# nnnagle/vq-vae

Measured on AMD Instinct MI355X. Metric: tiles/sec, higher is better.
Workload: dtype bf16

## Files before the change

### include/frl_hip.h

```cpp
#ifndef FRL_HIP_H
#define FRL_HIP_H

#include <stddef.h>
#include <stdint.h>

#ifdef __cplusplus
extern "C" {
#endif

typedef void* frl_stream_t;

enum { FRL_F32 = 0, FRL_BF16 = 1, FRL_F16 = 2  };
enum { FRL_ACT_NONE = 0, FRL_ACT_RELU = 1, FRL_ACT_SIGMOID = 2 };

int frl_version(void);
const char* frl_last_error(void);
int frl_device_arch(char* buf, int n);
int frl_kernel_timing_enable(int on);
int frl_kernel_timing_report(char* buf, int n);

size_t frl_pack_cache_table_bytes(void);
int frl_pack_cache_create(void* arena, size_t bytes);
int frl_pack_cache_destroy(int handle);
int frl_pack_cache_activate(int handle);
int frl_pack_cache_images(int handle);
int frl_pack_cache_refresh(int handle, frl_stream_t stream);

size_t frl_conv_workspace_bytes(int Cin, int Cout, int taps);
int frl_conv1x1_fwd(const void* x, const float* w, const float* bias, void* y, int64_t P, int Cin, int Cout, int act,
                    int dtype, void* ws, size_t ws_bytes, frl_stream_t stream);
int frl_conv1x1_bwd_data(const void* dy, const void* y, int act, const float* w, void* dx, int64_t P, int Cin, int Cout,
                         int dtype, void* ws, size_t ws_bytes, frl_stream_t stream);
int frl_conv1x1_bwd_data_add(const void* dy, const void* y, int act, const float* w, void* dx, const void* add, int64_t P,
                             int Cin, int Cout, int dtype, void* ws, size_t ws_bytes, frl_stream_t stream);
int frl_wgrad_set_max_workgroups(int n);
size_t frl_conv1x1_bwd_weight_workspace_bytes(int64_t P, int Cin, int Cout);
int frl_conv1x1_bwd_weight(const void* dy, const void* y, int act, const void* x, float* dw, float* dbias, int64_t P,
                           int Cin, int Cout, int dtype, void* ws, size_t ws_bytes, frl_stream_t stream);
int frl_conv_tap_bwd_weight(const void* dy, const void* y, int act, const void* x, float* dw, int64_t dso, int64_t dsi,
                            float* dbias, int64_t P, int Cin, int Cout, int HW, int T, int toff, int dtype, void* ws,
                            size_t ws_bytes, int flags, frl_stream_t stream);

int frl_conv3x3_fwd(const void* x, const float* w, const float* bias, void* y, int B, int H, int W, int Cin, int Cout,
                    int act, int dtype, void* ws, size_t ws_bytes, frl_stream_t stream);
int frl_conv3x3_fwd_gate_blend(const void* x, const float* w, const float* bias, const void* smoothed, const void* residual, void* gate,
                               void* out, int B, int H, int W, int Cin, int Cout, int dtype, void* ws, size_t ws_bytes,
                               frl_stream_t stream);
int frl_conv3x3_bwd_data(const void* dy, const void* y, int act, const float* w, void* dx, int B, int H, int W, int Cin,
                         int Cout, int dtype, void* ws, size_t ws_bytes, frl_stream_t stream);
int frl_conv3x3_bwd_data_fused(const void* dy, const void* y, int act, const float* w, void* dx, const void* add,
                               const void* sub_from, void* out2, int B, int H, int W, int Cin, int Cout, int dtype, void* ws,
                               size_t ws_bytes, frl_stream_t stream);
int frl_conv3x3_bwd_data_outmask(const void* dy, const void* y, int act, const float* w, void* dx, const void* out_y, int out_act, int B,
                                 int H, int W, int Cin, int Cout, int dtype, void* ws, size_t ws_bytes, frl_stream_t stream);
size_t frl_conv3x3_bwd_weight_workspace_bytes(int B, int H, int W, int Cin, int Cout);
int frl_conv3x3_bwd_weight(const void* dy, const void* y, int act, const void* x, float* dw, float* dbias, int B, int H,
                           int W, int Cin, int Cout, int dtype, void* ws, size_t ws_bytes, int flags, frl_stream_t stream);
int frl_conv3x3_wgrad_force_generic(int on);
int frl_conv3x3_tile32(int on);

int frl_groupnorm_fwd(const void* x, const float* gamma, const float* beta, void* y, float* mean, float* rstd, int B,
                      int HW, int C, int G, float eps, int relu, int dtype, frl_stream_t stream);
size_t frl_groupnorm_bwd_workspace_bytes(int B, int C, int G);
int frl_groupnorm_bwd(const void* dy, const void* x, const float* gamma, const float* beta, const float* mean,
                      const float* rstd, void* dx, float* dgamma, float* dbeta, int B, int HW, int C, int G, int relu,
                      int dtype, void* ws, size_t ws_bytes, frl_stream_t stream);

int frl_scalar_combine(const float* const* terms_host, const float* coef_host, int n, float* out, float* ok_out, frl_stream_t stream);
int frl_scalar_fanout(const float* g, const float* coef_host, int n, float* out, frl_stream_t stream);
int frl_scalar_combine_dev(const float* const* terms_host, const float* coef_host, const float* const* mult_host, int n, float* out,
                           float* ok_out, frl_stream_t stream);
int frl_scalar_combine_aux(const float* const* terms_host, const float* coef_host, const float* const* mult_host, const float* aux_coef_host,
                           int n, float* out, float* ok_out, float* aux_out, frl_stream_t stream);
int frl_scalar_fanout_dev(const float* g, const float* coef_host, const float* const* mult_host, int n, float* out, frl_stream_t stream);
int frl_scalar_fanout_guard(const float* g, const float* coef_host, const float* const* mult_host, const float* const* promise_host, int n,
                            float* out, int* flag, frl_stream_t stream);

int frl_encoder2_supported(int C0, int C1, int C2, int G1, int G2, int HW, int dtype);
size_t frl_encoder2_workspace_bytes(int B);
int frl_encoder2_fwd(const void* x, const float* w1, const float* g1, const float* b1, const float* w2, const float* g2, const float* b2,
                     void* z, float* stats, int B, int HW, float eps, void* ws, size_t ws_bytes, frl_stream_t stream);
int frl_encoder2_bwd(const void* x, const void* dz, const float* w1, const float* g1, const float* b1, const float* w2, const float* g2,
                     const float* b2, const float* stats, float* dw1, float* dg1, float* db1, float* dw2, float* dg2, float* db2,
                     int B, int HW, void* ws, size_t ws_bytes, frl_stream_t stream);

int frl_sobel_fwd(const void* x, void* g, int B, int H, int W, int C, int dtype, frl_stream_t stream);
int frl_sobel_bwd(const void* dg, void* dx, int B, int H, int W, int C, int dtype, frl_stream_t stream);
int frl_sobel_bwd_add(const void* dg, void* dx, const void* dx_add, int B, int H, int W, int C, int dtype, frl_stream_t stream);
int frl_edge_smooth_stencil_fwd(const void* x, const void* a_logit, const void* b_logit, void* smoothed, void* residual,
                                void* a_soft, void* b_soft, int B, int H, int W, int C, int R, int coarse_dilation,
                                int dtype, frl_stream_t stream);
int frl_edge_smooth_stencil_bwd(const void* d_smoothed, const void* x, const void* a_soft, const void* b_soft, void* dx,
                                void* da_logit, void* db_logit, const void* dx_add , int B, int H,
                                int W, int C, int R, int coarse_dilation, int dtype, frl_stream_t stream);
int frl_smooth_heads_supported(int C, int hidden, int rank, int dtype);
size_t frl_smooth_heads_workspace_bytes(int64_t npix);
int frl_smooth_heads_fwd(const void* x, const void* feat, const float* wa, const float* ba, const float* wb, const float* bb,
                         void* smoothed, void* residual, int B, int H, int W, int coarse_dilation, void* ws, size_t ws_bytes,
                         frl_stream_t stream);
size_t frl_smooth_heads_bwd_scratch_bytes(int64_t npix);
int frl_smooth_heads_force_gather(int on);
int frl_smooth_heads_bwd(const void* d_smoothed, const void* x, const void* feat, const float* wa, const float* ba, const float* wb,
                         const float* bb, const void* dx_add, void* dx, void* dfeat, float* dwa, float* dba, float* dwb, float* dbb,
                         void* scratch, size_t scratch_bytes, int B, int H, int W, int coarse_dilation, void* ws, size_t ws_bytes,
                         frl_stream_t stream);
int frl_smooth_heads_bwd_masked(const void* d_smoothed, const void* x, const void* feat, const float* wa, const float* ba, const float* wb,
                                const float* bb, const void* dx_add, void* dx, void* dfeat, float* dwa, float* dba, float* dwb, float* dbb,
                                void* scratch, size_t scratch_bytes, int B, int H, int W, int dil, int dfeat_relu, void* ws,
                                size_t ws_bytes, frl_stream_t stream);
int frl_film_fused_supported(int cond_dim, int hidden, int target_dim, int dtype);
size_t frl_film_fused_workspace_bytes(void);
int frl_film_fused_fwd(const void* z_type, const void* h, const float* w1g, const float* b1g, const float* w2g, const float* b2g,
                       const float* w1b, const float* b1b, const float* w2b, const float* b2b, void* z, void* gamma, void* beta, int B,
                       int T, int HW, void* ws, size_t ws_bytes, frl_stream_t stream);
int frl_film_fused_bwd(const void* z_type, const void* h, const void* dz, const float* w1g, const float* b1g, const float* w2g,
                       const float* b2g, const float* w1b, const float* b1b, const float* w2b, const float* b2b, void* dh, float* dw1g,
                       float* db1g, float* dw2g, float* db2g, float* dw1b, float* db1b, float* dw2b, float* db2b, int B, int T, int HW,
                       void* ws, size_t ws_bytes, frl_stream_t stream);
int frl_gate_blend_fwd(const void* smoothed, const void* residual, const void* gate_raw, float min_gate, void* out,
                       void* gate_out, int64_t n, int dtype, frl_stream_t stream);
int frl_gate_blend_bwd(const void* dout, const void* dgate_ext, const void* residual, const void* gate_raw, float min_gate,
                       void* d_residual, void* d_gate_raw, int64_t n, int dtype, frl_stream_t stream);
int frl_gate_blend_bwd_masked(const void* dout, const void* dgate_ext, const void* residual, const void* gate_raw, float min_gate,
                              void* d_residual, void* d_gate_raw, int64_t n, int dtype, int sigmoid_mask, frl_stream_t stream);

int frl_tcn_block_fwd(const void* x, const float* conv_w, const float* conv_b, const float* gn_w, const float* gn_b,
                      const float* gate_w, const float* gate_b, const float* proj_w, const float* proj_b, void* y,
                      int64_t npix, int HW, int T, int Cin, int Cout, int dilation, int G, float eps, int dtype, void* ws,
                      size_t ws_bytes, frl_stream_t stream);
size_t frl_tcn_block_bwd_workspace_bytes(int64_t npix, int Cout);
int frl_tcn_block_bwd(const void* x, const void* dy, const float* conv_w, const float* conv_b, const float* gn_w,
                      const float* gn_b, const float* gate_w, const float* gate_b, const float* proj_w,
                      const float* proj_b, void* dconv, void* dgpre, void* normed, void* dres, float* dgamma, float* dbeta,
                      int64_t npix, int HW, int T, int Cin, int Cout, int dilation, int G, float eps, int dtype, void* ws,
                      size_t ws_bytes, frl_stream_t stream);
int frl_tcn_block_bwd_data(const void* dconv, const void* dres, const float* conv_w, const float* proj_w, void* dx,
                           int64_t npix, int HW, int T, int Cin, int Cout, int dilation, int dtype, void* ws, size_t ws_bytes,
                           frl_stream_t stream);

int frl_tcn_block_bwd_fused_supported(int T, int Cin, int Cout, int G, int has_proj, int dtype);
size_t frl_tcn_block_bwd_fused_workspace_bytes(int64_t npix);
int frl_tcn_block_bwd_fused(const void* x, const void* dy, const float* conv_w, const float* conv_b, const float* gn_w,
                            const float* gn_b, const float* gate_w, const float* gate_b, void* dx, float* d_conv_w,
                            float* d_conv_b, float* d_gn_w, float* d_gn_b, float* d_gate_w, float* d_gate_b, int64_t npix,
                            int HW, int T, int dilation, int G, float eps, void* ws, size_t ws_bytes, frl_stream_t stream);

int frl_defer_begin(void);
int frl_defer_pending(void);
int frl_defer_destinations(void** out, int max);
int frl_defer_flush(frl_stream_t stream);
int frl_defer_abort(void);

int frl_tcn_hot_supported(int T, int Cin, int Cout, int G, int dilation, int has_proj, int dtype);
size_t frl_tcn_hot_fwd_workspace_bytes(void);
size_t frl_tcn_hot_bwd_workspace_bytes(int64_t npix);
int frl_tcn_hot_fwd(const void* x, const void* drop_mask, const float* conv_w, const float* conv_b, const float* gn_w, const float* gn_b,
                    const float* gate_w, const float* gate_b, void* y, int64_t npix, int HW, int dilation, float eps, void* ws,
                    size_t ws_bytes, frl_stream_t stream);
int frl_tcn_hot_bwd_nodx_supported(int64_t npix, int HW);
int frl_tcn_hot_bwd(const void* x, const void* drop_mask, const void* dy, const float* conv_w, const float* conv_b, const float* gn_w,
                    const float* gn_b, const float* gate_w, const float* gate_b, void* dx, float* d_conv_w, float* d_conv_b,
                    float* d_gn_w, float* d_gn_b, float* d_gate_w, float* d_gate_b, int64_t npix, int HW, int dilation,
                    float eps, void* ws, size_t ws_bytes, frl_stream_t stream);
size_t frl_tcn_chain_fwd_workspace_bytes(void);
int frl_tcn_chain_static_tiles(int on);
int frl_tcn_chain_fwd(const void* x, const float* const* conv_w, const float* const* conv_b, const float* const* gn_w,
                      const float* const* gn_b, const float* const* gate_w, const float* const* gate_b, const float* head_w,
                      const float* head_b, void* y1, void* y2, void* y3, void* h, int64_t npix, int HW, int Ch, float eps, void* ws,
                      size_t ws_bytes, frl_stream_t stream);
int frl_tcn_hot_bwd_head_supported(int64_t npix, int HW, int Ch);
size_t frl_tcn_hot_bwd_head_workspace_bytes(int64_t npix);
int frl_tcn_hot_bwd_head(const void* x, const void* dh, const float* head_w, int Ch, const float* conv_w, const float* conv_b,
                         const float* gn_w, const float* gn_b, const float* gate_w, const float* gate_b, void* dx, float* d_conv_w,
                         float* d_conv_b, float* d_gn_w, float* d_gn_b, float* d_gate_w, float* d_gate_b, int64_t npix, int HW,
                         int dilation, float eps, void* ws, size_t ws_bytes, frl_stream_t stream);
int frl_tcn_hot_force_generic_tiles(int on);
int frl_tcn_hot_bwd4_share(int variant, int share);

size_t frl_adamw_workspace_bytes(void);
int frl_adamw_clip_step(const void* desc_host, int ntensors, const void* chunks, const int* chunk_tensor, int nchunks, float max_norm,
                        float lr, double beta1, double beta2, float eps, int step, float* norm_out, const float* ok, int* counters,
                        const float* lr_dev, void* ws, size_t ws_bytes, frl_stream_t stream);
int frl_multi_tensor_scale_copy(const void* desc_host, int ntensors, const void* chunks, const int* chunk_tensor, int nchunks, float scale,
                                frl_stream_t stream);

int frl_film_modulate_fwd(const void* h, const void* gamma, const void* beta, void* out, int64_t B, int T, int64_t HW,
                          int C, int dtype, frl_stream_t stream);
int frl_film_modulate_bwd(const void* dout, const void* h, const void* gamma, void* dh, void* dgamma, void* dbeta,
// ... 96 lines not shown
```

### vq-vae_amd/csrc/pw_wgrad.hip

```cpp
#include "frl_common.hpp"
#include "frl_host.hpp"
#include "frl_reduce.hpp"
#include <type_traits>

#define WG_KP 64

template <typename T, int OBW, int IB>
__global__ __launch_bounds__(256) void pw_wgrad_kernel(
    const T* __restrict__ dY, const T* __restrict__ Ymask, int mask_act, const T* __restrict__ X,
    float* __restrict__ slab, int64_t P, int Cout, int Cin, int64_t rows_per_wg, int HW, int Tn, int toff,
    int use_tr, int64_t ldy) {
  typedef typename DT<T>::frag_t frag_t;
  typedef typename std::conditional<sizeof(T) == 2, bf16x8, f32x4>::type vec_t;
  constexpr int FE = DT<T>::FE;
  constexpr int VEC = DT<T>::VEC;
  extern __shared__ __attribute__((aligned(16))) char smem[];
  constexpr int CoP = OBW * 4 * 16, CiP = IB * 16;
  constexpr int pitchA = CoP + 8, pitchB = CiP + 8;
  constexpr int VPRA = CoP / VEC, VPRB = CiP / VEC;
  constexpr int NA = (WG_KP * VPRA + 255) / 256, NB = (WG_KP * VPRB + 255) / 256;
  T* ldsA = reinterpret_cast<T*>(smem);
  T* ldsB = ldsA + WG_KP * pitchA;
  const int tid = threadIdx.x, lane = tid & 63, wave = tid >> 6;
  const int r16 = lane & 15, kc = lane >> 4;
// ... 41 lines not shown
        ok = (t >= 0 && t < Tn);
      }
      const int64_t off = ok ? (p + shift) * (int64_t)Cin + c0 : 0;
      vec_t v = *reinterpret_cast<const vec_t*>(X + off);
      if (!ok) v = vec_t{};
      rb[u] = v;
    }
  };
  auto commit = [&]() {
#pragma unroll
    for (int u = 0; u < NA; ++u) {
      const int i = tid + u * 256;
      if (i >= nvA) continue;
      const int row = i / VPRA, c0 = (i % VPRA) * VEC;
      vec_t v = ra[u];
      if (Ymask != nullptr) {
#pragma unroll
        for (int e = 0; e < VEC; ++e) v[e] = from_f32<T>(to_f32(v[e]) * act_bwd_from_y(to_f32(rm[u][e]), mask_act));
      }
      *reinterpret_cast<vec_t*>(ldsA + (flatA ? i * VEC : row * pitchA + c0)) = v;
    }
#pragma unroll
    for (int u = 0; u < NB; ++u) {
      const int i = tid + u * 256;
      if (i >= WG_KP * VPRB) continue;
      const int row = i / VPRB, c0 = (i % VPRB) * VEC;
      *reinterpret_cast<vec_t*>(ldsB + row * pitchB + c0) = rb[u];
    }
  };
  if (fast && p_begin < p_end) fetch(p_begin);

  for (int64_t p0 = p_begin; p0 < p_end; p0 += WG_KP) {
    __syncthreads();
    if (fast) {
      commit();
    } else {
      for (int i = tid; i < WG_KP * VPRA; i += 256) {
        const int row = i / VPRA, c0 = (i % VPRA) * VEC;
        const int64_t p = p0 + row;
        float v[VEC];
#pragma unroll
        for (int e = 0; e < VEC; ++e) v[e] = 0.f;
        if (p < p_end && c0 < Cout) {
          const T* src = dY + p * ldy + c0;
#pragma unroll
          for (int e = 0; e < VEC; ++e)
            if (c0 + e < Cout) {
              v[e] = to_f32(src[e]);
              if (Ymask != nullptr) v[e] *= act_bwd_from_y(to_f32(Ymask[p * ldy + c0 + e]), mask_act);
            }
        }
        Vec<T>::store(ldsA + row * pitchA + c0, v);
      }
      for (int i = tid; i < WG_KP * VPRB; i += 256) {
        const int row = i / VPRB, c0 = (i % VPRB) * VEC;
        const int64_t p = p0 + row;
        float v[VEC];
#pragma unroll
        for (int e = 0; e < VEC; ++e) v[e] = 0.f;
        bool ok = p < p_end && c0 < Cin;
        if (ok && Tn > 1) {
          const int t = (int)((p / HW) % Tn) + toff;
          ok = (t >= 0 && t < Tn);
        }
        if (ok) {
          const T* src = X + (p + shift) * (int64_t)Cin + c0;
#pragma unroll
          for (int e = 0; e < VEC; ++e)
            if (c0 + e < Cin) v[e] = to_f32(src[e]);
        }
        Vec<T>::store(ldsB + row * pitchB + c0, v);
      }
    }
    __syncthreads();
    if (fast && p0 + WG_KP < p_end) fetch(p0 + WG_KP);
    if constexpr (FE == 8) {
      const bf16x8 ones = (r16 == 0) ? bf16x8{(bf16)1.f, (bf16)1.f, (bf16)1.f, (bf16)1.f, (bf16)1.f, (bf16)1.f, (bf16)1.f, (bf16)1.f}
                                     : bf16x8{(bf16)0.f, (bf16)0.f, (bf16)0.f, (bf16)0.f, (bf16)0.f, (bf16)0.f, (bf16)0.f, (bf16)0.f};
#pragma unroll
      for (int ks = 0; ks < WG_KP / 32; ++ks) {
        const int pix0 = ks * 32 + 8 * kc;
        bf16x8 bf[IB];
#pragma unroll
        for (int i = 0; i < IB; ++i) {
          const int ch0 = i * 16;
          if (use_tr) {
            const T* a0 = ldsB + (pix0 + (r16 >> 2)) * pitchB + ch0 + 4 * (r16 & 3);
            bf16x4 lo = __builtin_amdgcn_ds_read_tr16_b64_v4bf16(
                (bf16x4 __attribute__((address_space(3)))*)(a0));
            bf16x4 hi = __builtin_amdgcn_ds_read_tr16_b64_v4bf16(
                (bf16x4 __attribute__((address_space(3)))*)(a0 + 4 * pitchB));
            bf[i] = bf16x8{lo[0], lo[1], lo[2], lo[3], hi[0], hi[1], hi[2], hi[3]};
          } else {
#pragma unroll
            for (int j = 0; j < 8; ++j) bf[i][j] = ldsB[(pix0 + j) * pitchB + ch0 + r16];
          }
        }
#pragma unroll
        for (int o = 0; o < OBW; ++o) {
          const int ch0 = (wave * OBW + o) * 16;
          bf16x8 af;
          if (use_tr) {
            const T* a0 = ldsA + (pix0 + (r16 >> 2)) * pA + ch0 + 4 * (r16 & 3);
            bf16x4 lo = __builtin_amdgcn_ds_read_tr16_b64_v4bf16(
                (bf16x4 __attribute__((address_space(3)))*)(a0));
            bf16x4 hi = __builtin_amdgcn_ds_read_tr16_b64_v4bf16(
                (bf16x4 __attribute__((address_space(3)))*)(a0 + 4 * pA));
            af = bf16x8{lo[0], lo[1], lo[2], lo[3], hi[0], hi[1], hi[2], hi[3]};
          } else {
#pragma unroll
            for (int j = 0; j < 8; ++j) af[j] = ldsA[(pix0 + j) * pA + ch0 + r16];
          }
#pragma unroll
          for (int i = 0; i < IB; ++i) acc[o][i] = mfma16(af, bf[i], acc[o][i]);
          accb[o] = mfma16(af, ones, accb[o]);
        }
      }
    } else {
      const float ones = (r16 == 0) ? 1.f : 0.f;
#pragma unroll 4
      for (int ks = 0; ks < WG_KP / 4; ++ks) {
        const int pix = ks * 4 + kc;
        float bf[IB];
#pragma unroll
        for (int i = 0; i < IB; ++i) bf[i] = ldsB[pix * pitchB + i * 16 + r16];
#pragma unroll
        for (int o = 0; o < OBW; ++o) {
          const float af = ldsA[pix * pitchA + (wave * OBW + o) * 16 + r16];
#pragma unroll
          for (int i = 0; i < IB; ++i) acc[o][i] = mfma16(af, bf[i], acc[o][i]);
          accb[o] = mfma16(af, ones, accb[o]);
        }
      }
    }
  }
  float* my = slab + (int64_t)blockIdx.x * ((int64_t)Cout * Cin + Cout);
#pragma unroll
  for (int o = 0; o < OBW; ++o)
#pragma unroll
    for (int i = 0; i < IB; ++i)
#pragma unroll
      for (int r = 0; r < 4; ++r) {
        const int oc = (wave * OBW + o) * 16 + kc * 4 + r, ic = i * 16 + r16;
        if (oc < Cout && ic < Cin) my[(int64_t)oc * Cin + ic] = acc[o][i][r];
      }
  if (r16 == 0) {
#pragma unroll
    for (int o = 0; o < OBW; ++o)
#pragma unroll
      for (int r = 0; r < 4; ++r) {
        const int oc = (wave * OBW + o) * 16 + kc * 4 + r;
        if (oc < Cout) my[(int64_t)Cout * Cin + oc] = accb[o][r];
      }
  }
}


static int g_wgrad_max_wgs = 512;
static int wgrad_nwg(int64_t P) {
  int64_t n = (P + WG_KP - 1) / WG_KP;
  if (n > g_wgrad_max_wgs) n = g_wgrad_max_wgs;
  if (n < 1) n = 1;
  return (int)n;
}

template <typename T, int OBW, int IB>
static int launch_wgrad(const void* dy, const void* ymask, int mask_act, const void* x, float* ws, int64_t P,
                        int Cout, int Cin, int HW, int Tn, int toff, int use_tr, int64_t ldy, hipStream_t st) {
  const int nwg = wgrad_nwg(P);
  int64_t rows = (P + nwg - 1) / nwg;
  rows = (rows + WG_KP - 1) / WG_KP * WG_KP;
  const size_t lds = (size_t)WG_KP * ((OBW * 64 + 8) + (IB * 16 + 8)) * sizeof(T);
  auto kern = pw_wgrad_kernel<T, OBW, IB>;
  if (lds > 64 * 1024) FRL_HIP(hipFuncSetAttribute((const void*)kern, hipFuncAttributeMaxDynamicSharedMemorySize, (int)lds));
  FRL_LAUNCH_AS("pw_wgrad_kernel", kern, dim3(nwg), dim3(256), lds, st, (const T*)dy, (const T*)ymask, mask_act, (const T*)x, ws,
                     P, Cout, Cin, rows, HW, Tn, toff, use_tr, ldy);
  return frl_check_launch("pw_wgrad");
}

template <typename T>
static int dispatch_wgrad(const void* dy, const void* ymask, int mask_act, const void* x, float* ws, int64_t P,
                          int Cout, int Cin, int HW, int Tn, int toff, int use_tr, int64_t ldy, hipStream_t st) {
  const int ob = (Cout + 63) / 64;
  const int ib = (Cin + 15) / 16;
#define WG_CASE(O, I) return launch_wgrad<T, O, I>(dy, ymask, mask_act, x, ws, P, Cout, Cin, HW, Tn, toff, use_tr, ldy, st)
  if (ob <= 1) {
    if (ib <= 1) WG_CASE(1, 1);
    if (ib <= 2) WG_CASE(1, 2);
    if (ib <= 4) WG_CASE(1, 4);
    if (ib <= 8) WG_CASE(1, 8);
    if (ib <= 16) WG_CASE(1, 16);
  } else if (ob <= 2) {
    if (ib <= 1) WG_CASE(2, 1);
    if (ib <= 2) WG_CASE(2, 2);
    if (ib <= 4) WG_CASE(2, 4);
    if (ib <= 8) WG_CASE(2, 8);
  } else if (ob <= 4) {
    if (ib <= 1) WG_CASE(4, 1);
    if (ib <= 2) WG_CASE(4, 2);
    if (ib <= 4) WG_CASE(4, 4);
    if (ib <= 8) WG_CASE(4, 8);
  }
#undef WG_CASE
  return frl_fail(-2, "conv1x1_bwd_weight: unsupported (Cout, Cin) combination");
}

extern "C" {

int frl_wgrad_set_max_workgroups(int n) {
  const int was = g_wgrad_max_wgs;
  if (n >= 64 && n <= 4096) g_wgrad_max_wgs = n;
  return was;
}

size_t frl_conv1x1_bwd_weight_workspace_bytes(int64_t P, int Cin, int Cout) {
  return (size_t)wgrad_nwg(P) * ((size_t)Cout * Cin + Cout) * sizeof(float);
}

static int conv_tap_bwd_weight(const void* dy, const void* y, int act, const void* x, float* dw, int64_t dso,
                               int64_t dsi, float* dbias, int64_t P, int Cin, int Cout, int HW, int T, int toff,
                               int dtype, void* ws, size_t ws_bytes, int flags, hipStream_t stream, bool may_defer) {
  if (P <= 0) return frl_fail(-2, "bwd_weight: empty input");
  if (ws_bytes < frl_conv1x1_bwd_weight_workspace_bytes(P, Cin, Cout)) return frl_fail(-4, "bwd_weight: workspace too small");
  const void* ym = act != FRL_ACT_NONE ? y : nullptr;
  const int use_tr = (flags & 1) ? 0 : 1;
  const size_t esz = dtype == FRL_BF16 ? 2 : 4;
  for (int oc0 = 0; oc0 < Cout; oc0 += 256) {
    const int co = (Cout - oc0) < 256 ? (Cout - oc0) : 256;
    const char* dyp = (const char*)dy + (size_t)oc0 * esz;
    const char* ymp = ym ? (const char*)ym + (size_t)oc0 * esz : nullptr;
    int rc;
    if (dtype == FRL_F32) rc = dispatch_wgrad<float>(dyp, ymp, act, x, (float*)ws, P, co, Cin, HW, T, toff, 0, Cout, stream);
    else if (dtype == FRL_BF16) rc = dispatch_wgrad<bf16>(dyp, ymp, act, x, (float*)ws, P, co, Cin, HW, T, toff, use_tr, Cout, stream);
    else return frl_fail(-2, "bwd_weight: bad dtype");
    if (rc) return rc;
    const int64_t n = (int64_t)co * Cin + co;
    launch_slab_reduce_deferrable<float, WgradEpi>((const float*)ws, wgrad_nwg(P), n,
                                        WgradEpi{dw + (int64_t)oc0 * dso, dso, dsi, dbias ? dbias + oc0 : nullptr, co, Cin, (flags & 2) ? 1 : 0}, stream,
                                        may_defer && Cout <= 256 && (flags & 2) == 0);
  }
  return frl_check_launch("slab_reduce");
}

int frl_conv_tap_bwd_weight(const void* dy, const void* y, int act, const void* x, float* dw, int64_t dso,
                            int64_t dsi, float* dbias, int64_t P, int Cin, int Cout, int HW, int T, int toff,
                            int dtype, void* ws, size_t ws_bytes, int flags, hipStream_t stream) {
  const bool plain = dso == Cin && dsi == 1 && T == 1 && toff == 0;
  return conv_tap_bwd_weight(dy, y, act, x, dw, dso, dsi, dbias, P, Cin, Cout, HW, T, toff, dtype, ws, ws_bytes, flags, stream, plain);
}

int frl_conv1x1_bwd_weight(const void* dy, const void* y, int act, const void* x, float* dw, float* dbias,
                           int64_t P, int Cin, int Cout, int dtype, void* ws, size_t ws_bytes, hipStream_t stream) {
  return conv_tap_bwd_weight(dy, y, act, x, dw, Cin, 1, dbias, P, Cin, Cout, 1, 1, 0, dtype, ws, ws_bytes, 0, stream, true);
}

}
```

### vq-vae_amd/frl_hip/_lib.py

```python
from __future__ import annotations

import ctypes
import os
from ctypes import c_char_p, c_float, c_int, c_int64, c_size_t, c_void_p

_HERE = os.path.dirname(os.path.abspath(__file__))
LIB_PATH = os.path.join(_HERE, "libfrlhip_%s.so" % os.environ["FRL_HIP_LIB_TAG"] if os.environ.get("FRL_HIP_LIB_TAG") else "libfrlhip.so")

F32, BF16, F16 = 0, 1, 2
ACT_NONE, ACT_RELU, ACT_SIGMOID = 0, 1, 2

_lib = None


class FrlHipError(RuntimeError):
    pass


P, I, L, F, S, D = c_void_p, c_int, c_int64, c_float, c_size_t, ctypes.c_double
SIGNATURES = {
    "frl_version": (c_int, []),
    "frl_last_error": (c_char_p, []),
    "frl_device_arch": (c_int, [c_char_p, I]),
    "frl_kernel_timing_enable": (c_int, [I]),
    "frl_kernel_timing_report": (c_int, [c_char_p, I]),
    "frl_pack_cache_table_bytes": (S, []),
    "frl_pack_cache_create": (c_int, [P, S]),
    "frl_pack_cache_destroy": (c_int, [I]),
    "frl_pack_cache_activate": (c_int, [I]),
    "frl_pack_cache_images": (c_int, [I]),
    "frl_pack_cache_refresh": (c_int, [I, P]),
    "frl_conv_workspace_bytes": (S, [I, I, I]),
    "frl_conv1x1_fwd": (c_int, [P, P, P, P, L, I, I, I, I, P, S, P]),
    "frl_conv1x1_bwd_data": (c_int, [P, P, I, P, P, L, I, I, I, P, S, P]),
    "frl_conv1x1_bwd_data_add": (c_int, [P, P, I, P, P, P, L, I, I, I, P, S, P]),
    "frl_wgrad_set_max_workgroups": (c_int, [I]),
    "frl_conv3x3_wgrad_force_generic": (c_int, [I]),
    "frl_conv3x3_tile32": (c_int, [I]),
    "frl_conv1x1_bwd_weight_workspace_bytes": (S, [L, I, I]),
    "frl_conv1x1_bwd_weight": (c_int, [P, P, I, P, P, P, L, I, I, I, P, S, P]),
    "frl_conv_tap_bwd_weight": (c_int, [P, P, I, P, P, L, L, P, L, I, I, I, I, I, I, P, S, I, P]),
    "frl_vq_workspace_bytes": (S, [L, I, I]),
    "frl_vq_assign_fwd": (c_int, [P, P, L, I, I, P, P, P, P, I, P, S, P]),
    "frl_vq_prepared_bytes": (S, [I, I]),
    "frl_vq_prepare": (c_int, [P, L, I, I, I, P, S, P]),
    "frl_vq_stream_tiles": (c_int, [I]),
    "frl_vq_assign_fwd_prepared": (c_int, [P, P, P, L, I, I, P, P, P, P, I, P, S, P]),
    "frl_vq_bwd": (c_int, [P, P, P, P, P, P, P, F, L, I, I, P, P, P, I, P, S, P]),
    "frl_vq_ema_update": (c_int, [P, P, I, I, F, F, P, P, P, P, P]),
    "frl_vq_revive_dead_codes": (c_int, [P, P, L, P, L, I, I, ctypes.c_uint64, P, P, P, I, P]),
    "frl_groupnorm_fwd": (c_int, [P, P, P, P, P, P, I, I, I, I, F, I, I, P]),
    "frl_groupnorm_bwd_workspace_bytes": (S, [I, I, I]),
    "frl_groupnorm_bwd": (c_int, [P, P, P, P, P, P, P, P, P, I, I, I, I, I, I, P, S, P]),
    "frl_scalar_combine": (c_int, [P, P, I, P, P, P]),
    "frl_scalar_fanout": (c_int, [P, P, I, P, P]),
    "frl_scalar_combine_dev": (c_int, [P, P, P, I, P, P, P]),
    "frl_scalar_combine_aux": (c_int, [P, P, P, P, I, P, P, P, P]),
    "frl_scalar_fanout_dev": (c_int, [P, P, P, I, P, P]),
    "frl_scalar_fanout_guard": (c_int, [P, P, P, P, I, P, P, P]),
    "frl_encoder2_supported": (c_int, [I, I, I, I, I, I, I]),
    "frl_encoder2_workspace_bytes": (S, [I]),
    "frl_encoder2_fwd": (c_int, [P, P, P, P, P, P, P, P, P, I, I, F, P, S, P]),
    "frl_encoder2_bwd": (c_int, [P, P, P, P, P, P, P, P, P, P, P, P, P, P, P, I, I, P, S, P]),
    "frl_decoder_mse_fused_supported": (c_int, [I, I, I, I]),
    "frl_decoder_mse_workspace_bytes": (S, [L, I]),
    "frl_decoder_mse_fwd": (c_int, [P, P, P, P, P, P, P, P, P, L, I, P, S, P]),
    "frl_decoder_mse_bwd": (c_int, [P, P, P, P, P, P, P, P, P, P, P, P, P, P, L, I, P, S, P]),
    "frl_decoder_mse_onepass_bytes": (S, [L, I]),
    "frl_decoder_mse_fwd_bwd": (c_int, [P, P, P, P, P, P, P, P, P, P, P, S, P, P, L, I, P]),
    "frl_decoder_mse_reduce": (c_int, [P, I, P, P, P, P, I, P]),
    "frl_mse_workspace_bytes": (S, []),
    "frl_mse_fwd": (c_int, [P, P, P, L, I, P, I, P, S, P]),
    "frl_mse_bwd": (c_int, [P, P, P, P, P, L, I, P, I, P]),
    "frl_film_modulate_fwd": (c_int, [P, P, P, P, L, I, L, I, I, P]),
    "frl_film_modulate_bwd": (c_int, [P, P, P, P, P, P, L, I, L, I, I, P]),
    "frl_film_fused_supported": (c_int, [I, I, I, I]),
    "frl_film_fused_workspace_bytes": (S, []),
    "frl_film_fused_fwd": (c_int, [P] * 13 + [I, I, I, P, S, P]),
    "frl_film_fused_bwd": (c_int, [P] * 20 + [I, I, I, P, S, P]),
    "frl_gate_blend_fwd": (c_int, [P, P, P, F, P, P, L, I, P]),
    "frl_gate_blend_bwd": (c_int, [P, P, P, P, F, P, P, L, I, P]),
    "frl_mean_time_fwd": (c_int, [P, P, L, I, L, I, P]),
    "frl_add": (c_int, [P, P, F, P, L, I, P]),
    "frl_normalize_tiles": (c_int, [P, I, P, P, P, I, P, L, I, P]),
    "frl_gather_locations_fwd": (c_int, [P, L, L, L, I, I, I, P, L, P, I, P]),
    "frl_segment_sum_rows": (c_int, [P, P, P, L, I, P, L, I, P]),
    "frl_infonce_fwd": (c_int, [P, I, P, P, P, L, P, L, F, I, P, P, P, P, P, P]),
    "frl_infonce_pair_grads": (c_int, [P, I, P, P, P, P, L, L, F, I, P, P, P]),
    "frl_mutual_knn_max_points": (S, [I]),
    "frl_mutual_knn": (c_int, [P, I, I, P, P, F, I, P, P, P]),
    "frl_host_parallel_copy": (c_int, [P, P, S, I]),
    "frl_normalize_chunk_tiles": (c_int, [P, I, I, I, I, I, P, I, I, P, P, I, P, P]),
    "frl_conv3x3_fwd": (c_int, [P, P, P, P, I, I, I, I, I, I, I, P, S, P]),
    "frl_conv3x3_fwd_gate_blend": (c_int, [P, P, P, P, P, P, P, I, I, I, I, I, I, P, S, P]),
    "frl_conv3x3_bwd_data": (c_int, [P, P, I, P, P, I, I, I, I, I, I, P, S, P]),
    "frl_conv3x3_bwd_data_fused": (c_int, [P, P, I, P, P, P, P, P, I, I, I, I, I, I, P, S, P]),
    "frl_conv3x3_bwd_weight_workspace_bytes": (S, [I, I, I, I, I]),
    "frl_conv3x3_bwd_weight": (c_int, [P, P, I, P, P, P, I, I, I, I, I, I, P, S, I, P]),
    "frl_sobel_fwd": (c_int, [P, P, I, I, I, I, I, P]),
    "frl_sobel_bwd": (c_int, [P, P, I, I, I, I, I, P]),
    "frl_sobel_bwd_add": (c_int, [P, P, P, I, I, I, I, I, P]),
    "frl_edge_smooth_stencil_fwd": (c_int, [P, P, P, P, P, P, P, I, I, I, I, I, I, I, P]),
    "frl_edge_smooth_stencil_bwd": (c_int, [P, P, P, P, P, P, P, P, I, I, I, I, I, I, I, P]),
    "frl_smooth_heads_supported": (c_int, [I, I, I, I]),
    "frl_smooth_heads_workspace_bytes": (S, [L]),
    "frl_smooth_heads_bwd_scratch_bytes": (S, [L]),
    "frl_smooth_heads_force_gather": (c_int, [I]),
    "frl_smooth_heads_fwd": (c_int, [P, P, P, P, P, P, P, P, I, I, I, I, P, S, P]),
    "frl_smooth_heads_bwd": (c_int, [P, P, P, P, P, P, P, P, P, P, P, P, P, P, P, S, I, I, I, I, P, S, P]),
    "frl_tcn_block_fwd": (c_int, [P, P, P, P, P, P, P, P, P, P, L, I, I, I, I, I, I, F, I, P, S, P]),
    "frl_tcn_block_bwd_data": (c_int, [P, P, P, P, P, L, I, I, I, I, I, I, P, S, P]),
    "frl_tcn_block_bwd_workspace_bytes": (S, [L, I]),
    "frl_tcn_block_bwd_fused_supported": (c_int, [I, I, I, I, I, I]),
    "frl_tcn_block_bwd_fused_workspace_bytes": (S, [L]),
    "frl_tcn_block_bwd_fused": (c_int, [P, P, P, P, P, P, P, P, P, P, P, P, P, P, P, L, I, I, I, I, F, P, S, P]),
    "frl_adamw_workspace_bytes": (S, []),
    "frl_adamw_clip_step": (c_int, [P, I, P, P, I, F, F, D, D, F, I, P, P, P, P, P, S, P]),
    "frl_multi_tensor_scale_copy": (c_int, [P, I, P, P, I, F, P]),
    "frl_tcn_hot_supported": (c_int, [I, I, I, I, I, I, I]),
    "frl_tcn_hot_fwd_workspace_bytes": (S, []),
    "frl_tcn_hot_bwd_workspace_bytes": (S, [L]),
    "frl_tcn_hot_fwd": (c_int, [P, P, P, P, P, P, P, P, P, L, I, I, F, P, S, P]),
    "frl_tcn_hot_bwd": (c_int, [P, P, P, P, P, P, P, P, P, P, P, P, P, P, P, P, L, I, I, F, P, S, P]),
    "frl_tcn_hot_force_generic_tiles": (c_int, [I]),
    "frl_decoder_mse_bwd_subgroups": (c_int, [I]),
    "frl_tcn_hot_bwd4_share": (c_int, [I, I]),
    "frl_tcn_chain_static_tiles": (c_int, [I]),
    "frl_conv3x3_bwd_data_outmask": (c_int, [P, P, I, P, P, P, I, I, I, I, I, I, I, P, S, P]),
    "frl_gate_blend_bwd_masked": (c_int, [P, P, P, P, F, P, P, L, I, I, P]),
    "frl_smooth_heads_bwd_masked": (c_int, [P, P, P, P, P, P, P, P, P, P, P, P, P, P, P, S, I, I, I, I, I, P, S, P]),
    "frl_tcn_hot_bwd_head_supported": (c_int, [L, I, I]),
    "frl_tcn_hot_bwd_head_workspace_bytes": (S, [L]),
    "frl_tcn_hot_bwd_head": (c_int, [P, P, P, I, P, P, P, P, P, P, P, P, P, P, P, P, P, L, I, I, F, P, S, P]),
    "frl_defer_begin": (c_int, []),
    "frl_defer_pending": (c_int, []),
    "frl_defer_destinations": (c_int, [P, I]),
    "frl_defer_flush": (c_int, [P]),
    "frl_defer_abort": (c_int, []),
    "frl_tcn_hot_bwd_nodx_supported": (c_int, [L, I]),
    "frl_tcn_chain_fwd_workspace_bytes": (S, []),
    "frl_tcn_chain_fwd": (c_int, [P] * 13 + [L, I, I, F, P, S, P]),
    "frl_tcn_block_bwd": (c_int, [P, P, P, P, P, P, P, P, P, P, P, P, P, P, P, P, L, I, I, I, I, I, I, F, I, P, S, P]),
    "frl_decode_codes": (c_int, [P, P, P, L, I, I, I, P, P]),
    "frl_vicreg_workspace_bytes": (S, [L, I]),
    "frl_vicreg_fwd": (c_int, [P, L, I, I, F, F, F, F, P, P, P, P, S, P]),
    "frl_vicreg_bwd": (c_int, [P, P, P, P, L, I, I, F, F, F, F, P, P]),
    "frl_soft_nbr_fwd": (c_int, [P, P, P, P, L, I, F, F, I, P, P, P, P, P]),
    "frl_soft_nbr_bwd": (c_int, [P, P, P, P, P, L, I, P, P]),
    "frl_soft_nbr_gathered_fwd": (c_int, [P, I, P, I, I, P, P, P, P, P, P, L, I, I, F, F, I, P, P, P, P]),
    "frl_soft_nbr_gathered_bwd": (c_int, [P, I, P, I, I, P, P, P, P, P, P, L, I, I, F, F, I, P, P, P, P, P]),
}


def load():
    global _lib
    if _lib is not None:
        return _lib
    if not os.path.exists(LIB_PATH):
        raise FrlHipError(
            f"{LIB_PATH} not found: build it with `python vq-vae_amd/build.py` "
            "(hipcc --offload-arch=gfx950). There is no CPU fallback.")
    import torch
    lib = ctypes.CDLL(LIB_PATH)
    for name, (res, args) in SIGNATURES.items():
        fn = getattr(lib, name)
        fn.restype = res
        fn.argtypes = args
    _lib = lib
    return lib


def check(rc: int, what: str = "") -> None:
    if rc != 0:
        msg = load().frl_last_error()
        raise FrlHipError(f"{what} failed with code {rc}: {msg.decode() if msg else ''}")
```

### vq-vae_amd/frl_hip/ops.py

```python
from __future__ import annotations

import ctypes
from typing import Optional, Tuple

import torch

from . import _lib
from ._lib import ACT_NONE, ACT_RELU, ACT_SIGMOID, BF16, F32, check

_WS = {}

_TIMING = {"on": False, "events": {}}


def set_timing(on: bool) -> None:
    _TIMING["on"] = bool(on)
    _TIMING["events"] = {}


def timing_summary():
    torch.cuda.synchronize()
    return {k: (len(v), sum(a.elapsed_time(b) for a, b in v)) for k, v in _TIMING["events"].items()}


# ... 129 lines not shown
        raise _lib.FrlHipError(f"{name}: tensor must live on the GPU (no CPU fallback)")
    if not t.is_contiguous() or t.shape[-1] != c:
        raise ValueError(f"{name}: expected contiguous [..., {c}] rows, got {tuple(t.shape)} stride {t.stride()}")


def _chk_like(t: torch.Tensor, ref: torch.Tensor, name: str):
    if t.shape != ref.shape or t.dtype != ref.dtype or t.device != ref.device or not t.is_contiguous():
        raise ValueError(f"{name}: expected a contiguous {tuple(ref.shape)} {ref.dtype} tensor on {ref.device}, got "
                         f"{tuple(t.shape)} {t.dtype} stride {t.stride()}")


def _f32(t: Optional[torch.Tensor], name: str):
    if t is None:
        return None
    if t.dtype != torch.float32 or not t.is_contiguous() or not t.is_cuda:
        raise ValueError(f"{name}: parameters are passed as contiguous float32 CUDA tensors")
    return t


_DEFER = {"on": False, "keep": [], "dest": {}, "drop": set()}


class deferred_reductions:

    def __init__(self, params):
        self.params = list(params)

    def __enter__(self):
        check(_lib.load().frl_defer_begin(), "frl_defer_begin")
        _DEFER.update(keep=[], dest={}, drop=set(), on=True)
        return self

    def __exit__(self, et, ev, tb):
        lib = _lib.load()
        _DEFER["on"] = False
        keep, dest, drop = _DEFER["keep"], _DEFER["dest"], _DEFER["drop"]
        _DEFER.update(keep=[], dest={}, drop=set())
        if et is not None:
            lib.frl_defer_abort()
            return False
        try:
            import bisect
            buf = (ctypes.c_void_p * 512)()
            n = lib.frl_defer_destinations(ctypes.cast(buf, ctypes.c_void_p), 512)
            held = sorted((a, a + s.nbytes()) for a, s in dest.items())
            spans = sorted((g.data_ptr(), g.data_ptr() + g.numel() * g.element_size())
                           for g in (p.grad for p in self.params) if g is not None)
            for i in range(n):
                d = int(buf[i])
                k = bisect.bisect_right(held, (d, float("inf"))) - 1
                if k < 0 or not (held[k][0] <= d < held[k][1]):
                    raise RuntimeError("deferred_reductions: a parked gradient was not allocated by the kernel wrappers inside this block")
                if held[k][0] in drop:
                    continue
                k = bisect.bisect_right(spans, (d, float("inf"))) - 1
                if k < 0 or not (spans[k][0] <= d < spans[k][1]):
                    raise RuntimeError("deferred_reductions: a parked gradient is not the .grad of any parameter (autograd copied or summed "
                                       "it: a parameter used twice, a gradient accumulated into an existing .grad, or a gradient hook); "
                                       "the .grad of the parameters involved is now invalid: zero it, then run this backward without deferral")
        except Exception:
            lib.frl_defer_abort()
            raise
        rc = lib.frl_defer_flush(_stream())
        if rc < 0:
            check(rc, "frl_defer_flush")
        cur = torch.cuda.current_stream()
        for t in keep:
            t.record_stream(cur)
        for st in dest.values():
            torch.empty(0, dtype=torch.uint8, device=cur.device).set_(st).record_stream(cur)
        return False


def grad_empty(shape, device) -> torch.Tensor:
    g = torch.empty(shape, dtype=torch.float32, device=device)
    if _DEFER["on"]:
        st = g.untyped_storage()
        _DEFER["dest"][st.data_ptr()] = st
    return g


def discard(*grads) -> None:
    if _DEFER["on"]:
        for g in grads:
            if g is not None and g.untyped_storage().data_ptr() in _DEFER["dest"]:
                _DEFER["drop"].add(g.untyped_storage().data_ptr())


def workspace(nbytes: int, device) -> torch.Tensor:
    if _DEFER["on"]:
        ws = torch.empty(max(nbytes, 256), dtype=torch.uint8, device=device)
        _DEFER["keep"].append(ws)
        return ws
    key = (str(device), torch.cuda.current_stream().cuda_stream)
    ws = _WS.get(key)
    if ws is None or ws.numel() < nbytes:
        ws = torch.empty(max(nbytes, 1 << 20), dtype=torch.uint8, device=device)
        _WS[key] = ws
    return ws


@_timed("conv1x1_fwd")
def conv1x1_fwd(x: torch.Tensor, w: torch.Tensor, bias: Optional[torch.Tensor], act: int = ACT_NONE) -> torch.Tensor:
    cout, cin = w.shape[0], w.shape[1]
    _chk_rows(x, cin, "conv1x1_fwd.x")
    w = _f32(w.reshape(cout, cin), "w")
    y = torch.empty(x.shape[:-1] + (cout,), dtype=x.dtype, device=x.device)
    p = x.numel() // cin
    lib = _lib.load()
    ws = workspace(lib.frl_conv_workspace_bytes(cin, cout, 1), x.device)
    check(lib.frl_conv1x1_fwd(_p(x), _p(w), _p(_f32(bias, "bias")), _p(y), p, cin, cout, act, _dt(x), _p(ws), ws.numel(),
                              _stream()), "frl_conv1x1_fwd")
    return y


@_timed("conv1x1_bwd_data")
def conv1x1_bwd_data(dy: torch.Tensor, w: torch.Tensor, y: Optional[torch.Tensor] = None, act: int = ACT_NONE,
                     add: Optional[torch.Tensor] = None) -> torch.Tensor:
    cout, cin = w.shape[0], w.shape[1]
    _chk_rows(dy, cout, "conv1x1_bwd_data.dy")
    w = _f32(w.reshape(cout, cin), "w")
    dx = torch.empty(dy.shape[:-1] + (cin,), dtype=dy.dtype, device=dy.device)
    p = dy.numel() // cout
    lib = _lib.load()
    ws = workspace(lib.frl_conv_workspace_bytes(cin, cout, 1), dy.device)
    if add is not None:
        _chk_like(add, dx, "conv1x1_bwd_data.add")
        check(lib.frl_conv1x1_bwd_data_add(_p(dy), _p(y), act, _p(w), _p(dx), _p(add), p, cin, cout, _dt(dy), _p(ws), ws.numel(),
                                           _stream()), "frl_conv1x1_bwd_data_add")
        return dx
    check(lib.frl_conv1x1_bwd_data(_p(dy), _p(y), act, _p(w), _p(dx), p, cin, cout, _dt(dy), _p(ws), ws.numel(), _stream()),
          "frl_conv1x1_bwd_data")
    return dx


def _conv1x1_bwd_weight_impl(dy: torch.Tensor, x: torch.Tensor, y: Optional[torch.Tensor] = None, act: int = ACT_NONE,
                       want_bias: bool = True, scalar_frags: bool = False) -> Tuple[torch.Tensor, Optional[torch.Tensor]]:
    cout, cin = dy.shape[-1], x.shape[-1]
    _chk_rows(dy, cout, "bwd_weight.dy")
    _chk_rows(x, cin, "bwd_weight.x")
    p = dy.numel() // cout
    lib = _lib.load()
    nbytes = lib.frl_conv1x1_bwd_weight_workspace_bytes(p, cin, cout)
    ws = workspace(nbytes, dy.device)
    dw = grad_empty((cout, cin), dy.device)
    db = grad_empty((cout,), dy.device) if want_bias else None
    check(lib.frl_conv_tap_bwd_weight(_p(dy), _p(y), act, _p(x), _p(dw), cin, 1, _p(db), p, cin, cout, 1, 1, 0,
                                      _dt(dy), _p(ws), ws.numel(), 1 if scalar_frags else 0, _stream()),
          "frl_conv_tap_bwd_weight")
    return dw, db


conv1x1_bwd_weight = _timed("conv1x1_bwd_weight")(_conv1x1_bwd_weight_impl)


def vq_stream_tiles(nt: int) -> int:
    return int(_lib.load().frl_vq_stream_tiles(int(nt)))


@_timed("vq_prepare")
def vq_prepare(codebook: torch.Tensor, n_rows: int, dtype: torch.dtype, out: Optional[torch.Tensor] = None) -> torch.Tensor:
    k, d = codebook.shape
    cb = _f32(codebook, "codebook")
    lib = _lib.load()
    nbytes = lib.frl_vq_prepared_bytes(k, d)
    if out is None or out.numel() < nbytes or out.device != cb.device:
        out = torch.empty(nbytes, dtype=torch.uint8, device=cb.device)
    check(lib.frl_vq_prepare(_p(cb), int(n_rows), k, d, BF16 if dtype == torch.bfloat16 else F32, _p(out), out.numel(), _stream()),
          "frl_vq_prepare")
    return out


@_timed("vq_assign")
def vq_assign(z: torch.Tensor, codebook: torch.Tensor, prep: Optional[torch.Tensor] = None):
    k, d = codebook.shape
    _chk_rows(z, d, "vq_assign.z")
    cb = _f32(codebook, "codebook")
    n = z.numel() // d
    lib = _lib.load()
    ws = workspace(lib.frl_vq_workspace_bytes(n, k, d), z.device)
    idx = torch.empty(n, dtype=torch.int32, device=z.device)
    zq = torch.empty_like(z)
    stats = torch.empty(4, dtype=torch.float32, device=z.device)
    counts = torch.empty(k, dtype=torch.int32, device=z.device)
    if prep is not None and (prep.dtype != torch.uint8 or prep.device != z.device or prep.numel() < lib.frl_vq_prepared_bytes(k, d)):
        raise ValueError("vq_assign: prep is not a prepared-codebook image for this codebook")
    check(lib.frl_vq_assign_fwd_prepared(_p(z), _p(cb), _p(prep), n, k, d, _p(idx), _p(zq), _p(stats), _p(counts), _dt(z), _p(ws),
                                         ws.numel(), _stream()), "frl_vq_assign_fwd")
    return idx, zq, stats, counts


@_timed("vq_bwd")
def vq_bwd(g_out: Optional[torch.Tensor], z: torch.Tensor, codebook: torch.Tensor, idx: torch.Tensor,
           counts: torch.Tensor, gscale: Optional[torch.Tensor], beta: float, want_gz: bool = True,
           want_ge: bool = True, want_sums: bool = False, zq: Optional[torch.Tensor] = None):
    k, d = codebook.shape
    n = z.numel() // d
    lib = _lib.load()
    ws = workspace(lib.frl_vq_workspace_bytes(n, k, d), z.device)
    gz = torch.empty_like(z) if want_gz else None
    ge = grad_empty((k, d), z.device) if want_ge else None
    sums = torch.empty(k, d, dtype=torch.float32, device=z.device) if want_sums else None
    cb32 = _f32(codebook, "codebook")
    if _DEFER["on"]:
        _DEFER["keep"] += [t for t in (counts, gscale, cb32) if t is not None]
    check(lib.frl_vq_bwd(_p(g_out), _p(z), _p(zq), _p(cb32), _p(idx), _p(counts), _p(gscale), float(beta),
                         n, k, d, _p(gz), _p(ge), _p(sums), _dt(z), _p(ws), ws.numel(), _stream()), "frl_vq_bwd")
    return gz, ge, sums


def vq_ema_update(sums, counts, ema_count, ema_sum, codebook, decay: float, eps: float, ok: Optional[torch.Tensor] = None):
    k, d = codebook.shape
    if ok is not None and (ok.dtype != torch.float32 or not ok.is_cuda or ok.numel() < 1):
        raise ValueError("vq_ema_update: ok must be a float32 CUDA tensor")
    check(_lib.load().frl_vq_ema_update(_p(sums), _p(counts), k, d, float(decay), float(eps), _p(ema_count),
                                        _p(ema_sum), _p(codebook), _p(ok), _stream()), "frl_vq_ema_update")


def _mult_ptrs(mults, n):
    if mults is None or all(m is None for m in mults):
        return None
    for m in mults:
        if m is not None and (m.dtype != torch.float32 or m.numel() != 1 or not m.is_cuda):
            raise ValueError("scalar_combine: multipliers are float32 CUDA scalars")
    return (ctypes.c_void_p * n)(*[0 if m is None else m.data_ptr() for m in mults])


def scalar_combine(terms, coefs, mults=None, aux_coefs=None):
    n = len(terms)
    dev = terms[0].device
    for t in terms:
        if t.dtype != torch.float32 or t.numel() != 1 or not t.is_cuda:
            raise ValueError("scalar_combine: terms are float32 CUDA scalars")
    ptrs = (ctypes.c_void_p * n)(*[t.data_ptr() for t in terms])
    cf = (ctypes.c_float * n)(*[float(c) for c in coefs])
    out = torch.empty((), dtype=torch.float32, device=dev)
    ok = torch.empty(1, dtype=torch.float32, device=dev)
    if aux_coefs is None:
        check(_lib.load().frl_scalar_combine_dev(ptrs, cf, _mult_ptrs(mults, n), n, _p(out), _p(ok), _stream()), "frl_scalar_combine")
        return out, ok
    ac = (ctypes.c_float * n)(*[float(c) for c in aux_coefs])
    aux = torch.empty((), dtype=torch.float32, device=dev)
    check(_lib.load().frl_scalar_combine_aux(ptrs, cf, _mult_ptrs(mults, n), ac, n, _p(out), _p(ok), _p(aux), _stream()), "frl_scalar_combine_aux")
    return out, ok, aux


def scalar_fanout(g, coefs, mults=None, promises=None):
    n = len(coefs)
    cf = (ctypes.c_float * n)(*[float(c) for c in coefs])
    out = torch.empty(n, dtype=torch.float32, device=g.device)
    if promises is None or all(p is None for p in promises):
        check(_lib.load().frl_scalar_fanout_dev(_p(g), cf, _mult_ptrs(mults, n), n, _p(out), _stream()), "frl_scalar_fanout")
        return out
    for p in promises:
        if p is not None and (p.dtype != torch.float32 or p.numel() != 1 or p.device != g.device):
            raise ValueError("scalar_fanout: promises are float32 scalars on the gradient's device")
    pp = (ctypes.c_void_p * n)(*[0 if p is None else p.data_ptr() for p in promises])
    check(_lib.load().frl_scalar_fanout_guard(_p(g), cf, _mult_ptrs(mults, n), pp, n, _p(out), _p(_grad_scale_flag(g.device)), _stream()),
          "frl_scalar_fanout_guard")
    return out


_GRAD_SCALE_FLAG = {}


def _grad_scale_flag(device) -> torch.Tensor:
    device = torch.device(device)
    if device.index is None:
        device = torch.device(device.type, torch.cuda.current_device())
    flag = _GRAD_SCALE_FLAG.get(device)
    if flag is None:
        flag = _GRAD_SCALE_FLAG[device] = torch.zeros(1, dtype=torch.int32, device=device)
    return flag


def grad_scale_errors(device=None, reset: bool = True) -> bool:
    hit = False
    for dev, flag in _GRAD_SCALE_FLAG.items():
        if device is None or torch.device(device) == dev:
            hit |= bool(flag.item())
            if reset:
                flag.zero_()
    return hit


def check_grad_scale(device=None) -> None:
    if grad_scale_errors(device):
        raise RuntimeError("decoder_mse: a loss whose gradients were computed in the forward for a promised upstream gradient (grad_scale) "
                           "received a different one in the backward -- the decoder gradients of that step are wrongly scaled.  Scale the "
                           "loss through the promised coefficient, or switch the one-pass path off (VQVAE.onepass_decoder = False)")


def encoder2_supported(c0: int, c1: int, c2: int, g1: int, g2: int, hw: int, dtype) -> bool:
    return bool(_lib.load().frl_encoder2_supported(c0, c1, c2, g1, g2, hw, 1 if dtype == torch.bfloat16 else 0))


@_timed("encoder2_fwd")
def encoder2_fwd(x, w1, g1, b1, w2, g2, b2, eps: float = 1e-5):
    b, c = x.shape[0], x.shape[-1]
    hw = x.numel() // (b * c)
    _chk_rows(x, c, "encoder2.x")
    lib = _lib.load()
    z = torch.empty(x.shape[:-1] + (w2.shape[0],), dtype=x.dtype, device=x.device)
    stats = torch.empty(b, 32, dtype=torch.float32, device=x.device)
    ws = workspace(lib.frl_encoder2_workspace_bytes(b), x.device)
    check(lib.frl_encoder2_fwd(_p(x), _p(_f32(w1, "w1")), _p(_f32(g1, "g1")), _p(_f32(b1, "b1")), _p(_f32(w2, "w2")), _p(_f32(g2, "g2")),
# ... 889 lines not shown
```

Baseline: 107,300.

## Add thin-Cout 1x1 weight-gradient kernel with per-wave register-prefetch pipeline

Adds a specialized bf16 1x1 weight-gradient kernel for small output channel counts (Cout<=16, Cin<=64). Each of the eight waves works independently on its own slice of rows, with private LDS staging, a two-deep register prefetch ring and transposed LDS reads feeding MFMA. Per-wave partial sums are reduced in LDS before one slab write per workgroup. The generic kernel wastes most of its 256-channel-wide tile on such thin layers; the new path adds a dispatch condition and a second code path to maintain.

Measured after the change: 107,800, median of 6. No clear change (+0.4%).

```diff
diff --git a/include/frl_hip.h b/include/frl_hip.h
--- a/include/frl_hip.h
+++ b/include/frl_hip.h
@@ -34,6 +34,7 @@
 int frl_conv1x1_bwd_data_add(const void* dy, const void* y, int act, const float* w, void* dx, const void* add, int64_t P,
                              int Cin, int Cout, int dtype, void* ws, size_t ws_bytes, frl_stream_t stream);
 int frl_wgrad_set_max_workgroups(int n);
+int frl_wgrad_thin(int on);
 size_t frl_conv1x1_bwd_weight_workspace_bytes(int64_t P, int Cin, int Cout);
 int frl_conv1x1_bwd_weight(const void* dy, const void* y, int act, const void* x, float* dw, float* dbias, int64_t P,
                            int Cin, int Cout, int dtype, void* ws, size_t ws_bytes, frl_stream_t stream);
diff --git a/vq-vae_amd/csrc/pw_wgrad.hip b/vq-vae_amd/csrc/pw_wgrad.hip
--- a/vq-vae_amd/csrc/pw_wgrad.hip
+++ b/vq-vae_amd/csrc/pw_wgrad.hip
@@ -217,6 +217,125 @@
         const int oc = (wave * OBW + o) * 16 + kc * 4 + r;
         if (oc < Cout) my[(int64_t)Cout * Cin + oc] = accb[o][r];
       }
+  }
+}
+
+#define TH_KP 32
+#define TH_NW 8
+#define TH_D 2
+
+template <int IB>
+__global__ __launch_bounds__(TH_NW * 64, 4) void pw_wgrad_thin_kernel(
+    const bf16* __restrict__ dY, const bf16* __restrict__ X, float* __restrict__ slab, int64_t P, int Cout, int Cin) {
+  constexpr int pitchB = IB * 16 + 8;
+  constexpr int A_EL = TH_KP * 16 + 8;
+  constexpr int WB = (A_EL + TH_KP * pitchB) * 2;
+  static_assert(WB % 16 == 0 && WB >= (16 * IB * 16 + 16) * 4, "wave region");
+  __shared__ __attribute__((aligned(16))) char smem[TH_NW * WB];
+  const int tid = threadIdx.x, lane = tid & 63, wave = tid >> 6;
+  const int r16 = lane & 15, kc = lane >> 4;
+  bf16* ldsA = reinterpret_cast<bf16*>(smem + wave * WB);
+  bf16* ldsB = ldsA + A_EL;
+
+  const int64_t nt = (P + TH_KP - 1) / TH_KP;
+  const int64_t G = (int64_t)gridDim.x * TH_NW, g = (int64_t)blockIdx.x * TH_NW + wave;
+  const int64_t t_begin = g * nt / G, t_end = (g + 1) * nt / G;
+
+  const int VPR = Cin >> 3;
+  int xrow[IB], xlds[IB];
+  unsigned xoff[IB];
+#pragma unroll
+  for (int u = 0; u < IB; ++u) {
+    const int i = (lane + u * 64) % (TH_KP * VPR);
+    const int row = i / VPR, c0 = (i - row * VPR) * 8;
+    xrow[u] = row;
+    xoff[u] = row * Cin + c0;
+    xlds[u] = row * pitchB + c0;
+  }
+  const unsigned ae0 = (lane % (4 * Cout)) * 8;
+
+  struct Tile { bf16x8 a; bf16x4 ah; bf16x8 b[IB]; };
+  Tile ring[TH_D];
+  auto rows_of = [&](int64_t t) {
+    const int64_t left = t < t_end ? P - t * TH_KP : 0;
+    return left > TH_KP ? TH_KP : (int)left;
+  };
+  auto fetch = [&](Tile& r, int64_t t) {
+    const int nrows = rows_of(t), nval = nrows * Cout;
+    const int64_t p0 = nrows > 0 ? t * TH_KP : 0;
+    const bool a16 = ae0 + 8 <= nval, a8 = !a16 && ae0 + 4 <= nval;
+    const bf16* ap = dY + p0 * (int64_t)Cout;
+    r.a = *reinterpret_cast<const bf16x8*>(a16 ? ap + ae0 : dY);
+    r.ah = *reinterpret_cast<const bf16x4*>(ap + (a8 ? ae0 : 0));
+    const bf16* xp = X + p0 * (int64_t)Cin;
+#pragma unroll
+    for (int u = 0; u < IB; ++u) r.b[u] = *reinterpret_cast<const bf16x8*>(xp + (xrow[u] < nrows ? xoff[u] : 0));
+  };
+  auto commit = [&](const Tile& r, int64_t t) {
+    const int nrows = rows_of(t), nval = nrows * Cout;
+    bf16x8 v = r.a;
+    if (ae0 + 8 > nval) {
+      v = bf16x8{};
+      if (ae0 + 4 <= nval) { v[0] = r.ah[0]; v[1] = r.ah[1]; v[2] = r.ah[2]; v[3] = r.ah[3]; }
+    }
+    *reinterpret_cast<bf16x8*>(ldsA + ae0) = v;
+#pragma unroll
+    for (int u = 0; u < IB; ++u)
+      *reinterpret_cast<bf16x8*>(ldsB + xlds[u]) = xrow[u] < nrows ? r.b[u] : bf16x8{};
+  };
+
+  f32x4 acc[IB], accb = f32x4{0.f, 0.f, 0.f, 0.f};
+#pragma unroll
+  for (int i = 0; i < IB; ++i) acc[i] = f32x4{0.f, 0.f, 0.f, 0.f};
+  const bf16x8 ones = (r16 == 0) ? bf16x8{(bf16)1.f, (bf16)1.f, (bf16)1.f, (bf16)1.f, (bf16)1.f, (bf16)1.f, (bf16)1.f, (bf16)1.f}
+                                 : bf16x8{(bf16)0.f, (bf16)0.f, (bf16)0.f, (bf16)0.f, (bf16)0.f, (bf16)0.f, (bf16)0.f, (bf16)0.f};
+  const bf16* fa = ldsA + (8 * kc + (r16 >> 2)) * Cout + 4 * (r16 & 3);
+  const bf16* fb = ldsB + (8 * kc + (r16 >> 2)) * pitchB + 4 * (r16 & 3);
+
+#pragma unroll
+  for (int s = 0; s < TH_D; ++s) fetch(ring[s], t_begin + s);
+  for (int64_t t = t_begin; t < t_end; t += TH_D) {
+#pragma unroll
+    for (int s = 0; s < TH_D; ++s) {
+      commit(ring[s], t + s);
+      fetch(ring[s], t + s + TH_D);
+      bf16x4 lo = __builtin_amdgcn_ds_read_tr16_b64_v4bf16((bf16x4 __attribute__((address_space(3)))*)(fa));
+      bf16x4 hi = __builtin_amdgcn_ds_read_tr16_b64_v4bf16((bf16x4 __attribute__((address_space(3)))*)(fa + 4 * Cout));
+      const bf16x8 af = bf16x8{lo[0], lo[1], lo[2], lo[3], hi[0], hi[1], hi[2], hi[3]};
+      bf16x8 bf[IB];
+#pragma unroll
+      for (int i = 0; i < IB; ++i) {
+        lo = __builtin_amdgcn_ds_read_tr16_b64_v4bf16((bf16x4 __attribute__((address_space(3)))*)(fb + i * 16));
+        hi = __builtin_amdgcn_ds_read_tr16_b64_v4bf16((bf16x4 __attribute__((address_space(3)))*)(fb + i * 16 + 4 * pitchB));
+        bf[i] = bf16x8{lo[0], lo[1], lo[2], lo[3], hi[0], hi[1], hi[2], hi[3]};
+      }
+#pragma unroll
+      for (int i = 0; i < IB; ++i) acc[i] = mfma16(af, bf[i], acc[i]);
+      accb = mfma16(af, ones, accb);
+    }
+  }
+
+  const int n = Cout * Cin + Cout;
+  float* part = reinterpret_cast<float*>(smem + wave * WB);
+#pragma unroll
+  for (int i = 0; i < IB; ++i)
+#pragma unroll
+    for (int r = 0; r < 4; ++r) {
+      const int oc = kc * 4 + r, ic = i * 16 + r16;
+      if (oc < Cout && ic < Cin) part[oc * Cin + ic] = acc[i][r];
+    }
+  if (r16 == 0) {
+#pragma unroll
+    for (int r = 0; r < 4; ++r)
+      if (kc * 4 + r < Cout) part[Cout * Cin + kc * 4 + r] = accb[r];
+  }
+  __syncthreads();
+  float* my = slab + (int64_t)blockIdx.x * n;
+  for (int j = tid; j < n; j += TH_NW * 64) {
+    float s = 0.f;
+#pragma unroll
+    for (int w = 0; w < TH_NW; ++w) s += reinterpret_cast<const float*>(smem + w * WB)[j];
+    my[j] = s;
   }
 }
 
@@ -270,7 +389,33 @@
   return frl_fail(-2, "conv1x1_bwd_weight: unsupported (Cout, Cin) combination");
 }
 
+static int g_wgrad_thin = 1;
+static bool wgrad_thin_serves(const void* dy, const void* x, int64_t P, int Cout, int Cin) {
+  return g_wgrad_thin && Cout <= 16 && (Cout % 4) == 0 && (Cin % 8) == 0 && Cin <= 64 && P >= 2 &&
+         (reinterpret_cast<uintptr_t>(dy) % 16) == 0 && (reinterpret_cast<uintptr_t>(x) % 16) == 0;
+}
+static int launch_wgrad_thin(const void* dy, const void* x, float* ws, int64_t P, int Cout, int Cin, hipStream_t st) {
+  const int nwg = wgrad_nwg(P);
+#define TH_CASE(I)                                                                                                              \
+  FRL_LAUNCH_AS("pw_wgrad_thin_kernel", pw_wgrad_thin_kernel<I>, dim3(nwg), dim3(TH_NW * 64), 0, st, (const bf16*)dy, (const bf16*)x, \
+                ws, P, Cout, Cin)
+  switch ((Cin + 15) / 16) {
+    case 1: TH_CASE(1); break;
+    case 2: TH_CASE(2); break;
+    case 3: TH_CASE(3); break;
+    default: TH_CASE(4); break;
+  }
+#undef TH_CASE
+  return frl_check_launch("pw_wgrad_thin");
+}
+
 extern "C" {
+
+int frl_wgrad_thin(int on) {
+  const int was = g_wgrad_thin;
+  if (on == 0 || on == 1) g_wgrad_thin = on;
+  return was;
+}
 
 int frl_wgrad_set_max_workgroups(int n) {
   const int was = g_wgrad_max_wgs;
@@ -295,7 +440,9 @@
     const char* dyp = (const char*)dy + (size_t)oc0 * esz;
     const char* ymp = ym ? (const char*)ym + (size_t)oc0 * esz : nullptr;
     int rc;
-    if (dtype == FRL_F32) rc = dispatch_wgrad<float>(dyp, ymp, act, x, (float*)ws, P, co, Cin, HW, T, toff, 0, Cout, stream);
+    if (dtype == FRL_BF16 && use_tr && !ym && T == 1 && toff == 0 && dso == Cin && dsi == 1 && wgrad_thin_serves(dy, x, P, Cout, Cin))
+      rc = launch_wgrad_thin(dy, x, (float*)ws, P, Cout, Cin, stream);
+    else if (dtype == FRL_F32) rc = dispatch_wgrad<float>(dyp, ymp, act, x, (float*)ws, P, co, Cin, HW, T, toff, 0, Cout, stream);
     else if (dtype == FRL_BF16) rc = dispatch_wgrad<bf16>(dyp, ymp, act, x, (float*)ws, P, co, Cin, HW, T, toff, use_tr, Cout, stream);
     else return frl_fail(-2, "bwd_weight: bad dtype");
     if (rc) return rc;
diff --git a/vq-vae_amd/frl_hip/_lib.py b/vq-vae_amd/frl_hip/_lib.py
--- a/vq-vae_amd/frl_hip/_lib.py
+++ b/vq-vae_amd/frl_hip/_lib.py
@@ -35,6 +35,7 @@
     "frl_conv1x1_bwd_data": (c_int, [P, P, I, P, P, L, I, I, I, P, S, P]),
     "frl_conv1x1_bwd_data_add": (c_int, [P, P, I, P, P, P, L, I, I, I, P, S, P]),
     "frl_wgrad_set_max_workgroups": (c_int, [I]),
+    "frl_wgrad_thin": (c_int, [I]),
     "frl_conv3x3_wgrad_force_generic": (c_int, [I]),
     "frl_conv3x3_tile32": (c_int, [I]),
     "frl_conv1x1_bwd_weight_workspace_bytes": (S, [L, I, I]),
diff --git a/vq-vae_amd/frl_hip/ops.py b/vq-vae_amd/frl_hip/ops.py
--- a/vq-vae_amd/frl_hip/ops.py
+++ b/vq-vae_amd/frl_hip/ops.py
@@ -305,6 +305,10 @@
 
 
 conv1x1_bwd_weight = _timed("conv1x1_bwd_weight")(_conv1x1_bwd_weight_impl)
+
+
+def wgrad_thin(on: bool) -> bool:
+    return bool(_lib.load().frl_wgrad_thin(1 if on else 0))
 
 
 def vq_stream_tiles(nt: int) -> int:
```
